# mpieva/mapping-iterative-assembler

Hardware: AMD Instinct MI355X
Metric: reads aligned/sec per iteration (16.5kb mito ref, 100bp reads) (higher is better)
Workload: dtype int32; 1 GPU; configs[1]: 1000000 synthetic 100 bp reads per GPU vs mt311 (16619 bp, circular), matrix flat; step = reiterate_assembly + pop_smp + cull + consensus; pass-1 coordinates = true positions; reads_per_gpu=1000000, total_reads=1000000, consensus_len=16619, bytes_per_read=182

## Files before the change

mapping-iterative-assembler_amd/csrc/align_body.h:

```cpp
#pragma once
#include "mia_layout.h"

namespace mia {

struct AlignArgs {
  const uint8_t* ref_codes;
  int32_t ref_start;
  int32_t len1;
  const uint8_t* read_packed;
  int32_t len2;
  const int32_t* pssm;
  int32_t sg5;
  PackParams pk;
  uint32_t lds_sub;
  uint32_t trace_stride;
  int16_t* cols_out;
  uint32_t dbg;
};

struct AlignResult {
  int32_t score, abc, abr, aec;
  uint32_t status;
  int32_t aer;
};

template <int CPL>
struct PackBits {
  static constexpr int IB = (CPL == 4) ? 8 : 10;
  static constexpr int SH = IB + 2;
  static constexpr uint32_t IDXM = (1u << IB) - 1u;
};

template <class P, int CPL, bool LASTCOL = false>
struct WindowAligner {
  typedef typename P::U U;
  typedef typename P::M M;
  static constexpr int IB = PackBits<CPL>::IB, SH = PackBits<CPL>::SH;
  static constexpr uint32_t IDXM = PackBits<CPL>::IDXM;

  MIA_HD static inline __attribute__((always_inline)) AlignResult run(P& w, const AlignArgs& a) {
    const uint32_t OFF = (uint32_t)a.pk.off;
    const uint32_t UNAV = ((uint32_t)a.pk.unavail << SH) | IDXM;
    const U lane = w.lane();
    const int len1 = a.len1, len2 = a.len2;
    const uint32_t RS2 = (uint32_t)((len2 + 1) & ~1) * 2u;

    for (int e0 = 0; e0 < len2 * 5; e0 += WAVE) {
      U e = lane + (uint32_t)e0;
      M ok = e < (uint32_t)(len2 * 5);
      U r = w.udiv5(e);
      U c1 = e - r * 5u;
      U byte = w.gload_u8(a.read_packed, r >> 1, ok);
      U c2 = (byte >> ((r & 1u) << 2)) & 15u;
      U d = w.depth(r, (uint32_t)len2);
      U v = w.gload_i32(a.pssm, (d * 5u + c1) * 5u + c2, ok);
      w.lds_w16(U(a.lds_sub) + c1 * RS2 + r * 2u, v, ok);
    }
    w.lds_fence();

    U col[CPL], sub_addr[CPL], KC[CPL], QC[CPL];
    for (int j = 0; j < CPL; j++) {
      col[j] = lane * (uint32_t)CPL + (uint32_t)j;
      M in = col[j] < (uint32_t)len1;
      U code = w.sel(in, w.gload_u8(a.ref_codes, U((uint32_t)a.ref_start) + col[j], in), U(4u));
      sub_addr[j] = U(a.lds_sub) + code * RS2;
      KC[j] = (U(0u) - ((U((uint32_t)GOP) + (col[j] - 1u) * (uint32_t)GEP) << SH)) + (TR_COLGAP << IB) + (col[j] - 1u - IDXM);
      QC[j] = ((col[j] * (uint32_t)GEP) << SH) + (U(IDXM) - col[j]);
    }
    const uint32_t WDC = TR_DIAG << IB;
    const U unav = U(UNAV);

    U Sb[CPL], q[CPL], rrun[CPL], pend[CPL], pw[CPL];
    {
      const uint32_t rk = IDXM;
      for (int j = 0; j < CPL; j++) {
        pw[j] = w.lds_r32(sub_addr[j]);
        Sb[j] = w.sext_lo(pw[j]) + OFF;
        q[j] = (Sb[j] << SH) + QC[j];
        pend[j] = (Sb[j] << SH) + rk;
        rrun[j] = unav;
      }
      for (int j4 = 0; j4 < CPL; j4 += 4)
        w.tr_w32(col[j4], U((TR_DIAG << 6) * 0x01010101u), col[j4] < (uint32_t)a.trace_stride);
    }
    U colbest = U(0u), colrow = U(0u);
    auto last_col_update = [&](int r) __attribute__((always_inline)) {
      U v = U(0u);
      for (int j = 0; j < CPL; j++) v = w.sel(col[j] == (uint32_t)(len1 - 1), Sb[j], v);
      M up = v > colbest;
      colbest = w.sel(up, v, colbest);
      colrow = w.sel(up, U((uint32_t)r), colrow);
    };
    if (LASTCOL) last_col_update(0);

    for (int r = 1; r < ((a.dbg & 4u) ? 1 : len2); r++) {
      const int32_t fresh = a.sg5 ? -(GOP + GEP * (r + 1)) : 0;
      const uint32_t freshb = (uint32_t)(fresh + (int32_t)OFF);
      const uint32_t WS = freshb << SH;
      const uint32_t KR = (0u - ((uint32_t)(GOP + GEP * (r - 1)) << SH)) + (TR_ROWGAP << IB) + ((uint32_t)(r - 1) - IDXM);
      const uint32_t RK = ((uint32_t)(GEP * r) << SH) + (IDXM - (uint32_t)r);
      const uint32_t row_tr = (uint32_t)r * a.trace_stride;
      const bool hi = (r & 1) != 0;
      if (!hi)
        for (int j = 0; j < CPL; j++) pw[j] = w.lds_r32(sub_addr[j] + (uint32_t)r * 2u);

      U dleft = w.shr1(Sb[CPL - 1], U(freshb));
      U rleft = w.shr1_max(rrun[CPL - 1], unav);
      U u0 = w.shr1_max(q[CPL - 2], unav);
      U u1 = w.shr1_max(q[CPL - 1], unav);
      U g[CPL];
      g[0] = u0;
      g[1] = w.umax(u0, u1);
      for (int j = 2; j < CPL; j++) g[j] = w.umax(g[j - 1], q[j - 2]);
      U excl = w.shr1_max(w.scan_max(g[CPL - 1]), unav);

      U best[CPL], Snew[CPL];
      for (int j = 0; j < CPL; j++) {
        U diag = (j == 0) ? dleft : Sb[j - 1];
        U rl = (j == 0) ? rleft : rrun[j - 1];
        U Wd = (diag << SH) + WDC;
        U Wc = w.umax(excl, g[j]) + KC[j];
        U Wr = rl + KR;
        U m3 = w.umax3(Wd, Wc, Wr);
        best[j] = w.umax(m3, U(WS));
        U sub = hi ? w.sext_hi(pw[j]) : w.sext_lo(pw[j]);
        Snew[j] = (best[j] >> SH) + w.sel(m3 < WS, U(0u), sub);
      }
// ... 79 lines not shown
```

mapping-iterative-assembler_amd/csrc/mia_hip.hip:

```cpp
#include <hip/hip_runtime.h>
#include <atomic>
#include <hip/hip_ext.h>
#include <stdio.h>
#include <stdlib.h>
#include <string.h>

#include <algorithm>
#include <cmath>
#include <chrono>
#include <string>
#include <thread>
#include <vector>

#include "../../include/mia_hip.h"
#include "mia_comm.h"
#include "mia_consensus_kernels.h"
#include "mia_kernels.h"
#include "bandx_kernels.h"
#include "mia_pass1_kernels.h"
#include "mia_myers_kernels.h"
#include "mia_trim_kernels.h"
#include "mia_peak_kernels.h"
#include "mia_iter_kernels.h"
#include "mia_ma_region_kernels.h"

using namespace mia;

enum Stage { STG_TRACE = 0, STG_PLAIN, STG_FILTER, STG_BAND, STG_BX_PLAN, STG_BX_VALUES, STG_BX_TRACE, STG_TALLY, STG_PASS1, STG_MA_SELECT, STG_MA_RENDER, STG_COUNT };
static const char* const STAGE_NAMES[STG_COUNT] = {"k_align_quad", "k_align_quad_plain", "k_diag_filter", "k_band_align", "k_bx_plan",
                                                   "k_bx_values", "k_bx_trace", "k_tally_binned", "k_pass1", "k_ma_region_select",
                                                   "k_ma_region_render"};

constexpr int OPEN_WGS = 1024;
constexpr int64_t OPEN_SLAB_BYTES = (int64_t)MAX_READ * 64 * 12;
constexpr int CTRL_BINS = 0;
constexpr int CTRL_HDR = (3 * N_BINS + 2 + 1) & ~1;
constexpr int CTRL_FILTER = CTRL_HDR + PH_WORDS;
constexpr int CTRL_LKN = CTRL_FILTER + 4, CTRL_CULLF = CTRL_LKN + 1, CTRL_NEV = CTRL_CULLF + 1, CTRL_TFLAGS = CTRL_NEV + 1;
constexpr int CTRL_GENN = CTRL_TFLAGS + 2;
constexpr int CTRL_BXC = (CTRL_GENN + 1 + 63) & ~63;
constexpr int CTRL_WORDS = CTRL_BXC + BXC_WORDS;
constexpr int CTRL_C0 = CTRL_BINS + 3 * N_BINS, CTRL_CN = CTRL_WORDS - CTRL_C0;

#ifdef MIA_HIP_ALT_PATHS
static inline const char* alt_env(const char* name) { return getenv(name); }
#define ALT_KERNEL(k) ((const void*)(k))
#else
static inline const char* alt_env(const char*) { return nullptr; }
#define ALT_KERNEL(k) ((const void*)nullptr)
#endif

struct mia_hip_ctx {
  int device = 0;
  int cus = 1;
  std::string err;
  struct PoolBlock { void* p; size_t cap; bool lent; };
  std::vector<PoolBlock> pool;
// ... 26 lines not shown
  int min_len = 0;
  std::vector<int32_t> h_len;
  uint64_t* d_rplanes = nullptr; int rplane_words = 0;
  int32_t* d_umax = nullptr; bool umax_valid = false;
  uint8_t* d_ref = nullptr; int ref_cap = 0; int L = 0, wrap = 0; int explicit_win = 0; bool have_ref = false; bool aligned = false;
  bool ref_mostly_bases = true;
  bool ref_few_n = true;
  int64_t kh_entries = 0;

  int32_t *d_bin_of = nullptr, *d_list = nullptr, *d_wide_list = nullptr, *d_retry_list = nullptr;
  int32_t* d_bins = nullptr;
  int32_t* d_plan_hdr = nullptr;
  bool deferred = false;
  unsigned char* d_slabs[N_CPL] = {nullptr, nullptr, nullptr};
  unsigned char* d_slabs_retry[3] = {nullptr, nullptr, nullptr};
  unsigned char* d_quad_slabs = nullptr;
  int quad_wgs = 0;
  int grid_wgs = 0;
  int window_wgs[N_CPL] = {0, 0, 0};
  int64_t plain_retried = 0, plain_total = 0;
  bool wide_to_caller = false;
  int32_t* d_scratch = nullptr; int64_t scratch_cap = 0; int64_t* d_scratch_off = nullptr; int64_t scratch_off_cap = 0;
  int32_t* d_open_list = nullptr; int64_t open_cap = 0; unsigned char* d_slabs_open = nullptr; bool use_direct_open = true; int64_t direct_open_steps = 0;
  bool direct_open_now = false;

  int use_filter = 1;
  int32_t *d_kocc_cnt = nullptr, *d_kocc_pos = nullptr;
  uint64_t* d_planes = nullptr; int64_t plane_cap = 0;
  uint32_t* d_filter_n = nullptr; int64_t filter_proven = 0, filter_seen = 0;
  int use_banddp = 1;
  int32_t* d_left_list = nullptr; int64_t left_cap = 0;
  uint32_t* d_band_slabs = nullptr; int64_t band_slab_cap = 0;
  int64_t band_done = 0;

  bool bx_ok = false;
  int use_bx = 1, use_lanes = 1; bool bx_serial = false; uint32_t bx_dbg = 0;
  int32_t *d_bx_sub = nullptr, *d_bx_mrow = nullptr; int16_t *d_bx_loss = nullptr, *d_bx_dl = nullptr;
  int32_t bx_min_m = 0, bx_max_m = 0;
  uint32_t* d_refnib = nullptr; int64_t refnib_cap = 0;
  uint32_t* d_khash = nullptr; int32_t* d_khash_ovf = nullptr; uint32_t khash_cap = 0;
  KbPair* d_kbits = nullptr;
  int use_quick = 1; int64_t quick_steps = 0;
  uint32_t* d_prep_bar = nullptr; uint32_t prep_bar_count = 0; bool no_prep_fuse = false;
  uint32_t* d_bx_plan = nullptr; int32_t* d_bx_expect = nullptr; int32_t* d_bx_lists = nullptr; int64_t bx_cap = 0;
  BxCandRec* d_bx_cand = nullptr; int64_t cand_cap = 0, cand2_cap = 0; bool plan_split = true;
  BxCandRec* d_bx_cand2 = nullptr; int use_fine = 1;
// ... 83 lines not shown
  mia_hip_collectives coll{}; bool comm = false; int comm_ranks = 1, comm_rank = 0; std::string coll_name;
  unsigned long long* d_gather = nullptr;
  std::vector<int64_t> h_gather;
  int64_t ev_pad = 0;
  int64_t* d_lstage = nullptr; int64_t lstage_cap = 0;
  int64_t* d_lmine = nullptr; int64_t lmine_cap = 0;
  int64_t* d_lall = nullptr; int64_t lall_cap = 0;
  int32_t* d_scores_all = nullptr; int64_t scores_all_cap = 0;
};

static void read_alt_switches(mia_hip_ctx* ctx) {
  auto on = [](const char* name) { const char* v = alt_env(name); return v && atoi(v) != 0; };
  if (on("MIA_HIP_NO_DIAG_FILTER")) { ctx->use_filter = 0; ctx->use_bx = 0; }
  if (on("MIA_HIP_NO_BAND_DP")) { ctx->use_banddp = 0; ctx->use_bx = 0; }
  if (on("MIA_HIP_NO_BANDX")) ctx->use_bx = 0;
  if (on("MIA_HIP_NO_LANES")) ctx->use_lanes = 0;
  if (on("MIA_HIP_BX_SERIAL")) ctx->bx_serial = true;
  if (on("MIA_HIP_NO_PLAN_SPLIT")) ctx->plan_split = false;
  if (on("MIA_HIP_NO_FINE")) ctx->use_fine = 0;
  if (const char* v = alt_env("MIA_HIP_FINE")) ctx->use_fine = atoi(v);
  if (on("MIA_HIP_NO_QUICK_PLAN")) ctx->use_quick = 0;
  if (const char* v = alt_env("MIA_HIP_QUICK_PLAN")) ctx->use_quick = atoi(v);
  if (on("MIA_HIP_NO_DIRECT_OPEN")) ctx->use_direct_open = false;
  if (on("MIA_HIP_NO_PREP_FUSE")) ctx->no_prep_fuse = true;
  if (on("MIA_HIP_NO_SPEC")) ctx->no_spec = true;
  if (on("MIA_HIP_SPEC_TEST")) ctx->spec_force = true;
  if (on("MIA_HIP_NO_SIDE_BUCKETS")) ctx->no_side_buckets = true;
  if (on("MIA_HIP_NO_ZERO_COPY")) ctx->zero_copy = false;
  if (on("MIA_HIP_NO_EXT_EVENTS")) ctx->ext_events = 0u;
  if (on("MIA_HIP_FAKE_EVENT_OVERFLOW")) ctx->fake_event_overflow = true;
  if (on("MIA_HIP_CULL_SCAN")) ctx->cull_scan = true;
  if (on("MIA_HIP_TAIL_SCANS")) ctx->tail_scans = true;
  if (on("MIA_HIP_NO_CULL_RECORDS")) ctx->cull_with_records = false;
  if (on("MIA_HIP_NO_BINNED_TALLY")) ctx->use_binned_tally = 0;
  if (on("MIA_HIP_NO_LINEAR_TALLY")) ctx->no_linear_tally = true;
  if (on("MIA_HIP_SORT2_UNPACKED")) ctx->sort2_unpacked = true;
  if (on("MIA_HIP_TALLY_INLINE")) ctx->tally_defer = false;
  if (const char* v = alt_env("MIA_HIP_STRAND_SPLIT")) ctx->tally_strand_split = atoi(v) != 0;
  if (on("MIA_HIP_NO_TALLY_RUNS")) ctx->tally_runs = false;
  if (on("MIA_HIP_NO_TALLY_RALL")) ctx->tally_rall = false;
  if (on("MIA_HIP_MYERS_NO_LANES")) ctx->myers_no_lanes = true;
  if (on("MIA_HIP_MYERS_NO_OND")) ctx->myers_no_ond = true;
  if (const char* v = alt_env("MIA_HIP_DEBUG_SKIP")) ctx->dbg = (uint32_t)atoi(v);
  if (const char* v = alt_env("MIA_HIP_BX_DEBUG")) ctx->bx_dbg = (uint32_t)atoi(v);
}

// ... 232 lines not shown
static void pack_reads(int64_t n, const char* bases, const int64_t* offsets, const uint32_t* roff, const uint16_t* len, uint8_t* packed) {
  uint8_t lut[256];
  for (int c = 0; c < 256; c++) lut[c] = base_code((char)c);
  auto range = [&](int64_t lo, int64_t hi) {
    for (int64_t i = lo; i < hi; i++) {
      const unsigned char* s = reinterpret_cast<const unsigned char*>(bases) + offsets[i];
      uint8_t* d = packed + roff[i];
      const int l = len[i];
      int k = 0;
      for (; k + 1 < l; k += 2) d[k >> 1] = (uint8_t)(lut[s[k]] | (lut[s[k + 1]] << 4));
      if (k < l) d[k >> 1] = lut[s[k]];
    }
  };
  int T = (int)std::thread::hardware_concurrency();
  if (const char* e = getenv("MIA_HIP_THREADS")) T = atoi(e);
  T = std::max(1, std::min(std::min(T, 32), (int)(n / 16384) + 1));
  if (T == 1) { range(0, n); return; }
  std::vector<std::thread> th;
  for (int t = 1; t < T; t++) th.emplace_back(range, n * t / T, n * (t + 1) / T);
  range(0, n / T);
  for (auto& x : th) x.join();
}

extern "C" int mia_hip_upload_reads(mia_hip_ctx* ctx, int64_t n, const char* bases, const int64_t* offsets, const uint8_t* rc,
                                    const uint8_t* strand_known, const int32_t* as, const int32_t* ae) {
  if (!ctx || n < 0 || (n > 0 && (!bases || !offsets || !rc || !strand_known || !as || !ae))) return MIA_HIP_ERR_ARG;
  if (n >= (int64_t)1 << 31) { ctx->err = "more than 2^31 reads per context"; return MIA_HIP_ERR_ARG; }
  HIPCHK(hipSetDevice(ctx->device));
  std::vector<uint32_t> roff((size_t)n);
  std::vector<uint16_t> len((size_t)n);
  uint64_t total = 0;
  int max_len = 1;
  for (int64_t i = 0; i < n; i++) {
    int64_t l = offsets[i + 1] - offsets[i];
    if (l < 1 || l > MIA_HIP_MAX_READ) { ctx->err = "read length outside 1..256 (INIT_ALN_SEQ_LEN)"; return MIA_HIP_ERR_ARG; }
    roff[i] = (uint32_t)total;
    len[i] = (uint16_t)l;
    if (l > max_len) max_len = (int)l;
    total += (uint64_t)(((l + 1) / 2 + 3) & ~3);
    if (total >= ((uint64_t)1 << 32)) { ctx->err = "packed read store exceeds 4 GiB per context"; return MIA_HIP_ERR_ARG; }
  }
  std::vector<uint8_t> packed((size_t)total + 8, 0);
  pack_reads(n, bases, offsets, roff.data(), len.data(), packed.data());
  ctx->max_len = max_len;
  ctx->min_len = max_len;
  ctx->h_len.assign(len.begin(), len.end());
// ... 14 lines not shown
  rcx |= dev_alloc(ctx, &ctx->d_cols, (size_t)n * stride);
  rcx |= dev_alloc(ctx, &ctx->d_bin_of, (size_t)n);
  rcx |= dev_alloc(ctx, &ctx->d_umax, (size_t)n);
  ctx->rplane_words = (max_len + 63) >> 6;
  rcx |= dev_alloc(ctx, &ctx->d_rplanes, (size_t)n * 2 * ctx->rplane_words + 2);
  rcx |= dev_alloc(ctx, &ctx->d_list, (size_t)n + 4 * N_BINS);
  rcx |= dev_alloc(ctx, &ctx->d_wide_list, (size_t)n);
  rcx |= dev_alloc(ctx, &ctx->d_retry_list, (size_t)n);
  rcx |= dev_alloc(ctx, &ctx->d_slot, (size_t)n);
  rcx |= dev_alloc(ctx, &ctx->d_partial, (size_t)(n / 256 + n / 4096 + 8));
  rcx |= dev_alloc(ctx, &ctx->d_drop_f, (size_t)n);
  rcx |= dev_alloc(ctx, &ctx->d_drop_b, (size_t)n);
  ctx->n_slots = 2 * n + 16;
  rcx |= dev_alloc(ctx, &ctx->d_slot_dropped, (size_t)ctx->n_slots);
  rcx |= dev_alloc(ctx, &ctx->d_back_slot, (size_t)n) | dev_alloc(ctx, &ctx->d_front_slot0, (size_t)n);
  rcx |= dev_alloc(ctx, &ctx->ri.flen, (size_t)n) | dev_alloc(ctx, &ctx->ri.blen, (size_t)n) | dev_alloc(ctx, &ctx->ri.actf, (size_t)n) |
         dev_alloc(ctx, &ctx->ri.trec, (size_t)n * 16);
  ctx->slot_cap = 2 * n + 16;
  rcx |= dev_alloc(ctx, &ctx->si.reclen, (size_t)ctx->slot_cap) | dev_alloc(ctx, &ctx->si.recact, (size_t)ctx->slot_cap) | dev_alloc(ctx, &ctx->si.writer, (size_t)ctx->slot_cap) |
         dev_alloc(ctx, &ctx->si.mult, (size_t)ctx->slot_cap);
  ctx->lk.cap = (int32_t)std::min<int64_t>(n + 16, (int64_t)1 << 20);
  if (ctx->lk.cap > (int32_t)LINK_NONE - 1) ctx->lk.cap = (int32_t)LINK_NONE - 1;
  rcx |= dev_alloc(ctx, &ctx->lk.rec, (size_t)ctx->lk.cap * 4);
  if (rcx) return MIA_HIP_ERR_NOMEM;
  HIPCHK(hipMemcpyAsync(ctx->d_packed, packed.data(), packed.size(), hipMemcpyHostToDevice, ctx->stream));
  HIPCHK(hipMemcpyAsync(ctx->d_roff, roff.data(), (size_t)n * 4, hipMemcpyHostToDevice, ctx->stream));
  HIPCHK(hipMemcpyAsync(ctx->d_len, len.data(), (size_t)n * 2, hipMemcpyHostToDevice, ctx->stream));
  HIPCHK(hipMemcpyAsync(ctx->d_rc, rc, (size_t)n, hipMemcpyHostToDevice, ctx->stream));
  HIPCHK(hipMemcpyAsync(ctx->d_sk, strand_known, (size_t)n, hipMemcpyHostToDevice, ctx->stream));
  HIPCHK(hipMemcpyAsync(ctx->d_as, as, (size_t)n * 4, hipMemcpyHostToDevice, ctx->stream));
  HIPCHK(hipMemcpyAsync(ctx->d_ae, ae, (size_t)n * 4, hipMemcpyHostToDevice, ctx->stream));
  HIPCHK(hipMemsetAsync(ctx->d_score, 0, (size_t)n * 4, ctx->stream));
  HIPCHK(hipMemsetAsync(ctx->d_status, 0, (size_t)n * 4, ctx->stream));
  HIPCHK(hipMemsetAsync(ctx->d_abr, 0, (size_t)n * 2, ctx->stream));
  HIPCHK(hipMemsetAsync(ctx->d_slot_dropped, 0, (size_t)ctx->n_slots, ctx->stream));
  HIPCHK(hipMemsetAsync(ctx->d_back_slot, 0xFF, (size_t)n * 8, ctx->stream));
  HIPCHK(hipMemsetAsync(ctx->d_front_slot0, 0xFF, (size_t)n * 8, ctx->stream));
  HIPCHK(hipMemsetAsync(ctx->d_drop_f, 0, (size_t)n, ctx->stream));
  HIPCHK(hipMemsetAsync(ctx->d_drop_b, 0, (size_t)n, ctx->stream));
  HIPCHK(hipStreamSynchronize(ctx->stream));
  ReadSet& r = ctx->rs;
  r.n = n; r.packed = ctx->d_packed; r.roff = ctx->d_roff; r.len = ctx->d_len; r.rc = ctx->d_rc; r.sk = ctx->d_sk;
  r.as = ctx->d_as; r.ae = ctx->d_ae; r.score = ctx->d_score; r.refstart = ctx->d_refstart; r.abr = ctx->d_abr;
  r.status = ctx->d_status; r.cols = ctx->d_cols; r.stride = stride;
  if (ctx->d_order) { (void)hipFree(ctx->d_order); ctx->d_order = nullptr; }
  if (ctx->d_order2) { (void)hipFree(ctx->d_order2); ctx->d_order2 = nullptr; }
// ... 200 lines not shown
  }
  RefInfo ref{ctx->d_ref, ctx->L, ctx->wrap, ctx->explicit_win};
  if (stage_begin(ctx, STG_TRACE, on)) return hipErrorOutOfMemory;
  launch_k(k_align_window<CPL>, dim3(grid), dim3(64), 0, on ? on : ctx->stream, stop, ctx->rs, ref, ctx->d_pssm, ctx->packs.p[ci], list,
           count, slabs, slab, ctx->d_wide_list, ctx->d_bins + 3 * N_BINS, ctx->dbg, dev_range);
  stage_end(ctx, STG_TRACE, on);
  return hipGetLastError();
}

static int bx_join_and_retry(mia_hip_ctx* ctx) {
  if (!ctx->bx_pending_join) return MIA_HIP_OK;
  ctx->bx_pending_join = false;
  const int32_t* range = ctx->d_plan_hdr + PH_RETRY2;
  const int cols = ctx->max_len + 2 * REALIGN_BUFFER + 2;
  const bool aside = ctx->bx_planner_aside;
  if (!aside || ctx->dp_aside) HIPCHK(hipStreamWaitEvent(ctx->stream, ctx->ev_join, 0));
  HIPCHK(hipStreamWaitEvent(ctx->stream, ctx->ev_join3, 0));
  hipEvent_t stop = (aside && (ctx->ext_events & 8u)) ? ctx->ev_fork : nullptr;
  ctx->align_end_signalled = stop != nullptr;
  hipError_t e;
  if (ctx->direct_open_now) {
    RefInfo ref{ctx->d_ref, ctx->L, ctx->wrap, ctx->explicit_win};
    if (stage_begin(ctx, STG_TRACE)) return MIA_HIP_ERR_NOMEM;
    launch_k(k_align_open, dim3(OPEN_WGS), dim3(64), 0, ctx->stream, stop, ctx->rs, ref, (const int32_t*)ctx->d_pssm, ctx->packs, (const int32_t*)ctx->d_open_list,
             (const uint32_t*)(ctx->d_bx_ctr + (size_t)BXC_OPEN * BXC_STRIDE), ctx->d_slabs_open, (int64_t)OPEN_SLAB_BYTES, ctx->d_wide_list, ctx->d_bins + 3 * N_BINS, ctx->dbg,
             (const int32_t*)ctx->d_retry2, (const uint32_t*)(range + 1));
    stage_end(ctx, STG_TRACE);
    e = hipGetLastError();
    if (e != hipSuccess) { ctx->err = std::string("k_align_open launch: ") + hipGetErrorString(e); return MIA_HIP_ERR_DEVICE; }
    return MIA_HIP_OK;
  }
  e = cols <= 64 * 4 ? launch_window<4>(ctx, 0, ctx->d_retry2, 0, range, nullptr, aside, stop)
    : cols <= 64 * 8 ? launch_window<8>(ctx, 1, ctx->d_retry2, 0, range, nullptr, aside, stop)
                     : launch_window<12>(ctx, 2, ctx->d_retry2, 0, range, nullptr, aside, stop);
  if (e != hipSuccess) { ctx->err = std::string("k_align_window (band retry list) launch: ") + hipGetErrorString(e); return MIA_HIP_ERR_DEVICE; }
  if (aside) {
    if (!ctx->planner_end_signalled) HIPCHK(hipEventRecord(ctx->ev_join, ctx->stream2));
    ctx->planner_end_signalled = false;
    HIPCHK(hipStreamWaitEvent(ctx->stream, ctx->ev_join, 0));
  }
  return MIA_HIP_OK;
}

static int align_all(mia_hip_ctx* ctx);
static bool tally_is_binned(const mia_hip_ctx* ctx);
static int comm_pre_cull_enqueue(mia_hip_ctx* ctx, const int32_t* d_wide_count);
static bool comm_pre_cull_collect(mia_hip_ctx* ctx);

extern "C" int mia_hip_realign(mia_hip_ctx* ctx, const char* new_ref, int32_t ref_len, int circular) {
// ... 233 lines not shown
      bd.rplanes = bd.umax ? ctx->d_rplanes : nullptr;
      bd.rplane_words = ctx->rplane_words;
      bd.plan = ctx->d_bx_plan; bd.expect = ctx->d_bx_expect; bd.lists = ctx->d_bx_lists; bd.list_stride = ctx->bx_cap; bd.ctr = ctx->d_bx_ctr;
      const bool split = ctx->plan_split;
      const bool fork_by_launch = (ctx->ext_events & 1u) && new_flow && !(ctx->dbg & 256u);
      bd.cand = nullptr; bd.cand_n = ctx->d_bx_ctr + (size_t)BXC_CAND * BXC_STRIDE;
      bd.cand2 = nullptr; bd.cand2_n = ctx->d_bx_ctr + (size_t)BXC_CAND2 * BXC_STRIDE;
      int64_t rejects_before = 0;
      for (int k = 1; k < BXF_KINDS; k++) rejects_before += ctx->bx_last[BXC_FAIL0 + k];
      const bool fine = split && ctx->use_fine && (ctx->use_fine > 1 || !ctx->flat || n >= 4000000 || !ctx->ref_mostly_bases || rejects_before * 20 > n);
      if (split) {
        if (n > ctx->cand_cap) {
          if (dev_alloc(ctx, &ctx->d_bx_cand, (size_t)n)) return MIA_HIP_ERR_NOMEM;
          ctx->cand_cap = n;
        }
        if (fine && n > ctx->cand2_cap) {
          if (dev_alloc(ctx, &ctx->d_bx_cand2, (size_t)n)) return MIA_HIP_ERR_NOMEM;
          ctx->cand2_cap = n;
        }
        bd.cand = ctx->d_bx_cand;
        if (fine) bd.cand2 = ctx->d_bx_cand2;
      }
      const int last_phase = split ? (fine ? 3 : 2) : 0;
      {
        int64_t lr = 0;
        for (int k = 1; k < BXF_KINDS; k++) lr += ctx->bx_last[BXC_FAIL0 + k];
        const bool many_early = !ctx->ref_mostly_bases || lr * 20 > n;
        planner_head_first = new_flow && ctx->deferred && many_early && !(ctx->dbg & 256u);
        const bool plain_wanted = many_early;
        direct_open = new_flow && ctx->deferred && ctx->use_direct_open && !plain_wanted && !planner_head_first && !(ctx->dbg & 256u) &&
                      !(ctx->bx_dbg & (4u | 8u));
      }
      bd.open = nullptr; bd.open_n = ctx->d_bx_ctr + (size_t)BXC_OPEN * BXC_STRIDE;
      ctx->direct_open_now = direct_open;
      if (direct_open) {
        if (n > ctx->open_cap) { if (dev_alloc(ctx, &ctx->d_open_list, (size_t)n)) return MIA_HIP_ERR_NOMEM; ctx->open_cap = n; }
        if (!ctx->d_slabs_open && hipMalloc((void**)&ctx->d_slabs_open, (size_t)OPEN_SLAB_BYTES * OPEN_WGS) != hipSuccess) return MIA_HIP_ERR_NOMEM;
        bd.open = ctx->d_open_list;
        ctx->direct_open_steps++;
      }
      if (!fine && ctx->use_fine < 2) bd.tab.maxw = 32;
      const bool quick = split && new_flow && want_bits && !(ctx->bx_dbg & 32u) && bd.umax != nullptr &&
                         (!fine || n >= 2000000 || ctx->use_quick > 1);
      bd.qlist = nullptr; bd.qlist_n = ctx->d_filter_n + 1; bd.mark_all = 0; bd.to_late = 0; bd.qch = 4;
      bool plan_launched = false;
      const bool fork_at_quick = quick && ctx->deferred && direct_open && !fine && !planner_head_first && !(ctx->bx_dbg & (4u | 8u));
      bd.kb = KmerBits{quick ? ctx->d_kbits : nullptr, ctx->L};
      const bool quick_lds = quick && words * 24 <= 38 * 1024;
      bd.plane_words = (int32_t)(quick_lds ? words : 0);
      if (quick) {
        if (n > ctx->left_cap) { if (dev_alloc(ctx, &ctx->d_left_list, (size_t)n)) return MIA_HIP_ERR_NOMEM; ctx->left_cap = n; }
        bd.qlist = ctx->d_left_list;
        ctx->quick_steps++;
      }
      if (stage_begin(ctx, STG_BX_PLAN)) return MIA_HIP_ERR_NOMEM;
      {
        const int32_t* in_list = quick ? ctx->d_left_list : nullptr;
        const dim3 pb(256);
        const int nwords = (ctx->max_len + 63) >> 6;
        const bool one_launch = quick && !fine;
        if (quick) {
          bd.qch = (n >= 4000000 && words * 24 <= 16 * 1024) ? BX_QCH : 4;
          const dim3 pg((unsigned)((n + 256 * bd.qch - 1) / (256 * bd.qch)));
          hipEvent_t done = (fork_at_quick && fork_by_launch) ? ctx->ev_fork : nullptr;
          const int32_t* in_list = nullptr;
#define MIA_PLAN(NWV, PHV) launch_k(k_bx_plan<NWV, PHV>, pg, pb, (size_t)(bx_quick_lds_words(bd.qch) * 8 + (PHV == 5 ? words * 24 : 0)), ctx->stream, done, ctx->rs, ref, rp, kh, (int64_t)wrap, bd, in_list, (const uint32_t*)(ctx->d_filter_n + 1), n, ctx->d_bin_of)
          if (quick_lds) { switch (nwords) { case 1: MIA_PLAN(1, 5); break; case 2: MIA_PLAN(2, 5); break; case 3: MIA_PLAN(3, 5); break; default: MIA_PLAN(4, 5); break; } }
          else { switch (nwords) { case 1: MIA_PLAN(1, 4); break; case 2: MIA_PLAN(2, 4); break; case 3: MIA_PLAN(3, 4); break; default: MIA_PLAN(4, 4); break; } }
#undef MIA_PLAN
          bd.mark_all = 1;
          if (fork_at_quick) {
            if (!fork_by_launch) HIPCHK(hipEventRecord(ctx->ev_fork, ctx->stream));
            bd.to_late = 1;
          }
        }
        const int phase_first = (split && !one_launch) ? 1 : 0, phase_last = one_launch ? 0 : last_phase;
        plan_launched = true;
        for (int phase = phase_first; phase <= phase_last; phase++) {
          const dim3 pg(phase >= 2 ? (unsigned)std::min<int64_t>((n + 255) / 256, 1024) : (unsigned)(one_launch ? std::min<int64_t>((n + 255) / 256, 256) : (n + 255) / 256));
          hipEvent_t done = (fork_by_launch && phase == phase_last && !planner_head_first && !fork_at_quick) ? ctx->ev_fork : nullptr;
#define MIA_PLAN(NWV, PHV) launch_k(k_bx_plan<NWV, PHV>, pg, pb, 0, ctx->stream, done, ctx->rs, ref, rp, kh, (int64_t)wrap, bd, in_list, (const uint32_t*)(ctx->d_filter_n + 1), n, ctx->d_bin_of)
#define MIA_PLAN_NW(PHV) switch (nwords) { case 1: MIA_PLAN(1, PHV); break; case 2: MIA_PLAN(2, PHV); break; case 3: MIA_PLAN(3, PHV); break; default: MIA_PLAN(4, PHV); break; }
          switch (phase) {
            case 0: if (one_launch) { MIA_PLAN_NW(6) } else { MIA_PLAN_NW(0) } break;
            case 1: MIA_PLAN_NW(1) break;
            case 2: MIA_PLAN_NW(2) break;
            default: MIA_PLAN_NW(3) break;
          }
#undef MIA_PLAN_NW
#undef MIA_PLAN
        }
        bd.to_late = 0;
      }
      stage_end(ctx, STG_BX_PLAN);
      HIPCHK(hipGetLastError());
      if (planner_head_first) {
        hipLaunchKernelGGL(k_plan_count, dim3(gb), dim3(tb), 0, ctx->stream, ctx->rs, ref, ctx->packs, 1, filtered, filtered, ctx->d_bin_of, d_count, ctx->d_filter_n);
        hipLaunchKernelGGL(k_plan_scan, dim3(1), dim3(512), 0, ctx->stream, d_count, d_off, ctx->d_plan_hdr, 0, ctx->d_list);
        launch_k(k_plan_fill, dim3(gb), dim3(tb), 0, ctx->stream, fork_by_launch ? ctx->ev_fork : nullptr, n, (const int32_t*)ctx->d_bin_of, (const int32_t*)d_off, d_cursor, ctx->d_list);
        HIPCHK(hipGetLastError());
      }
      if (!(ctx->dbg & 256u)) {
        if (new_flow) {
          hipStream_t vs = (ctx->deferred && !fork_at_quick) ? ctx->stream : ctx->stream2;
// ... 946 lines not shown
```

mapping-iterative-assembler_amd/csrc/mia_kernels.h:

```cpp
#pragma once
#include <hip/hip_runtime.h>
#include <stdint.h>

#include "align_body.h"
#include "align_body_quad.h"
#include "align_body_quad_plain.h"
#include "diag_filter.h"
#include "band_body.h"
#include "mia_layout.h"
#include "wave_dev.h"

namespace mia {

constexpr int N_CPL = 3;
constexpr int BIN_WIDE = N_CPL;
constexpr int BIN_QUAD0 = BIN_WIDE + 1;
constexpr int N_BINS = BIN_QUAD0 + MAX_READ + 1;
constexpr int SUB_LDS_BYTES = MAX_READ * 10;

struct ReadSet {
  int64_t n;
  const uint8_t* packed;
  const uint32_t* roff;
  const uint16_t* len;
// ... 340 lines not shown
    a.trace_stride = (uint32_t)((l1 + 3) & ~3);
    a.cols_out = rs.cols + (int64_t)i * rs.stride;
    a.dbg = dbg;
    AlignResult r = WindowAligner<DevWave, CPL>::run(wave, a);
    if (wave.lane() == 0) {
      if (r.status & ST_ESCAPE) {
        int p = atomicAdd(wide_count, 1);
        wide_list[p] = i;
      } else {
        rs.score[i] = r.score;
        rs.refstart[i] = s;
        rs.abr[i] = (int16_t)r.abr;
        rs.as[i] = r.abc + s;
        rs.ae[i] = r.aec + s;
      }
      rs.status[i] = r.status;
    }
    wave.lds_fence();
  }
}

__global__ __launch_bounds__(64) void k_align_open(ReadSet rs, RefInfo ref, const int32_t* pssm2, PackSet ps, const int32_t* list, const uint32_t* count_p,
                                                    unsigned char* trace_slabs, int64_t slab_bytes, int32_t* wide_list, int32_t* wide_count, uint32_t dbg,
                                                    const int32_t* list_b, const uint32_t* count_b_p) {
  __shared__ __attribute__((aligned(16))) unsigned char lds_raw[SUB_LDS_BYTES];
  const int count_a = (int)*count_p, count = count_a + (list_b ? (int)*count_b_p : 0);
  __builtin_amdgcn_s_setprio(3);
  DevWave wave(lds_raw, trace_slabs + (int64_t)blockIdx.x * slab_bytes);
  for (int w = blockIdx.x; w < count; w += gridDim.x) {
    const int i = w < count_a ? list[w] : list_b[w - count_a];
    if (!rs.sk[i]) { if (wave.lane() == 0) rs.status[i] = ST_SKIPPED; continue; }
    AlignArgs a;
    int s, l1;
    const int len2 = rs.len[i];
    read_window(ref, rs.as[i], rs.ae[i], len2, &s, &l1);
    const int ci = classify(len2, l1, ps, 0);
    if (ci == BIN_WIDE) {
      if (wave.lane() == 0) { const int q = atomicAdd(wide_count, 1); wide_list[q] = i; }
      continue;
    }
    a.ref_codes = ref.codes;
    a.ref_start = s;
    a.len1 = l1;
    a.read_packed = rs.packed + rs.roff[i];
    a.len2 = len2;
    a.pssm = pssm2 + (rs.rc[i] ? PSSM_WORDS : 0);
    a.sg5 = 1;
    a.pk = ps.p[ci];
    a.lds_sub = 0;
    a.trace_stride = (uint32_t)((l1 + 3) & ~3);
    a.cols_out = rs.cols + (int64_t)i * rs.stride;
    a.dbg = dbg;
    AlignResult r;
    if (ci == 0) r = WindowAligner<DevWave, 4>::run(wave, a);
    else if (ci == 1) r = WindowAligner<DevWave, 8>::run(wave, a);
    else r = WindowAligner<DevWave, 12>::run(wave, a);
    if (wave.lane() == 0) {
      if (r.status & ST_ESCAPE) {
        const int q = atomicAdd(wide_count, 1);
        wide_list[q] = i;
      } else {
        rs.score[i] = r.score;
        rs.refstart[i] = s;
        rs.abr[i] = (int16_t)r.abr;
        rs.as[i] = r.abc + s;
        rs.ae[i] = r.aec + s;
      }
      rs.status[i] = r.status;
    }
    wave.lds_fence();
  }
}

__global__ __launch_bounds__(64, 4) void k_align_quad(ReadSet rs, RefInfo ref, const int32_t* pssm2, PackParams pk, const int32_t* list,
                                                    int32_t n_quads, unsigned char* trace_slabs, int64_t slab_bytes,
                                                    int32_t* wide_list, int32_t* wide_count, int32_t* retry_list, int32_t* retry_count,
                                                    int32_t band, uint32_t dbg, const int32_t* dev_range) {
  extern __shared__ __attribute__((aligned(16))) unsigned char lds_raw[];
  if (dev_range) { list += dev_range[0]; n_quads = dev_range[1]; }
// ... 211 lines not shown
```

mapping-iterative-assembler_amd/csrc/wave_dev.h:

```cpp
#pragma once
#include <hip/hip_runtime.h>
#include <stdint.h>

#include "mia_layout.h"

namespace mia {

constexpr int DPP_ROW_SHR = 0x110;
constexpr int DPP_WAVE_SHR1 = 0x138;
constexpr int DPP_ROW_BCAST15 = 0x142;
constexpr int DPP_ROW_BCAST31 = 0x143;

struct DevWave {
  typedef uint32_t U;
  typedef bool M;
  unsigned char* lds;
  unsigned char* trace;

  __device__ __forceinline__ DevWave(unsigned char* l, unsigned char* t) : lds(l), trace(t) {}

  __device__ __forceinline__ U lane() const { return __builtin_amdgcn_mbcnt_hi(~0u, __builtin_amdgcn_mbcnt_lo(~0u, 0u)); }

  __device__ __forceinline__ U shr1(U x, U fill) const {
    return (U)__builtin_amdgcn_update_dpp((int)fill, (int)x, DPP_WAVE_SHR1, 0xF, 0xF, false);
// ... 122 lines not shown
  __device__ __forceinline__ U lds_r32m(U off, M ok) const { return ok ? *reinterpret_cast<const uint32_t*>(lds + off) : 0u; }
  __device__ __forceinline__ static U gload_u32(const uint32_t* p, U i, M ok) { return ok ? p[i] : 0u; }
  __device__ __forceinline__ static void gstore_u32(uint32_t* p, U i, U v, M ok) { if (ok) p[i] = v; }
  __device__ __forceinline__ U tr_r16(U off, M ok) const {
    return ok ? (U)__hip_atomic_load(reinterpret_cast<const uint16_t*>(trace + off), __ATOMIC_RELAXED, __HIP_MEMORY_SCOPE_AGENT) : 0u;
  }
  __device__ __forceinline__ void tr_w32(U off, U v, M ok) const { if (ok) *reinterpret_cast<uint32_t*>(trace + off) = v; }
  __device__ __forceinline__ U tr_r8(U off, M ok) const {
    return ok ? (U)__hip_atomic_load(trace + off, __ATOMIC_RELAXED, __HIP_MEMORY_SCOPE_AGENT) : 0u;
  }
  __device__ __forceinline__ void tr_fence() const {
    __builtin_amdgcn_fence(__ATOMIC_RELEASE, "workgroup");
    __builtin_amdgcn_wave_barrier();
    __builtin_amdgcn_fence(__ATOMIC_ACQUIRE, "workgroup");
  }
  __device__ __forceinline__ void sched_fence() const { __builtin_amdgcn_sched_barrier(0); }
  __device__ __forceinline__ void lds_fence() const {
    __builtin_amdgcn_fence(__ATOMIC_RELEASE, "workgroup");
    __builtin_amdgcn_wave_barrier();
    __builtin_amdgcn_fence(__ATOMIC_ACQUIRE, "workgroup");
  }
};

}
```

Baseline: 1.440 billion reads/s.

## Keep open-window traceback matrix in LDS and batch PSSM staging loads

The open-window alignment kernel now uses dynamic shared memory sized from the device limit, and narrow-bin reads whose traceback fits are written and read from LDS instead of a global slab. The substitution-staging loop batches eight rows of global loads before the LDS writes so more loads are in flight, and the per-row LDS substitution read is prefetched one row ahead. Global slabs are now sized by max read length and allocated at read upload, and an env flag forces all reads through the open path. The larger LDS footprint per workgroup may lower occupancy, and extra registers for the batching and prefetch may add register pressure.

```diff
diff --git a/mapping-iterative-assembler_amd/csrc/align_body.h b/mapping-iterative-assembler_amd/csrc/align_body.h
--- a/mapping-iterative-assembler_amd/csrc/align_body.h
+++ b/mapping-iterative-assembler_amd/csrc/align_body.h
@@ -31,7 +31,7 @@
   static constexpr uint32_t IDXM = (1u << IB) - 1u;
 };
 
-template <class P, int CPL, bool LASTCOL = false>
+template <class P, int CPL, bool LASTCOL = false, bool ALONE = false>
 struct WindowAligner {
   typedef typename P::U U;
   typedef typename P::M M;
@@ -45,32 +45,50 @@
     const int len1 = a.len1, len2 = a.len2;
     const uint32_t RS2 = (uint32_t)((len2 + 1) & ~1) * 2u;
 
-    for (int e0 = 0; e0 < len2 * 5; e0 += WAVE) {
-      U e = lane + (uint32_t)e0;
-      M ok = e < (uint32_t)(len2 * 5);
-      U r = w.udiv5(e);
-      U c1 = e - r * 5u;
-      U byte = w.gload_u8(a.read_packed, r >> 1, ok);
-      U c2 = (byte >> ((r & 1u) << 2)) & 15u;
-      U d = w.depth(r, (uint32_t)len2);
-      U v = w.gload_i32(a.pssm, (d * 5u + c1) * 5u + c2, ok);
-      w.lds_w16(U(a.lds_sub) + c1 * RS2 + r * 2u, v, ok);
+    U col[CPL], code[CPL];
+    auto load_codes = [&]() __attribute__((always_inline)) {
+      for (int j = 0; j < CPL; j++) {
+        col[j] = lane * (uint32_t)CPL + (uint32_t)j;
+        M in = col[j] < (uint32_t)len1;
+        code[j] = w.sel(in, w.gload_u8(a.ref_codes, U((uint32_t)a.ref_start) + col[j], in), U(4u));
+      }
+    };
+    if (ALONE) load_codes();
+
+    constexpr int SUB_BATCH = ALONE ? 8 : 1;
+    for (int e0 = 0; e0 < len2 * 5; e0 += SUB_BATCH * WAVE) {
+      U sr[SUB_BATCH], sc1[SUB_BATCH], sbyte[SUB_BATCH], sv[SUB_BATCH];
+      for (int k = 0; k < SUB_BATCH; k++) {
+        U e = lane + (uint32_t)(e0 + k * WAVE);
+        M ok = e < (uint32_t)(len2 * 5);
+        sr[k] = w.udiv5(e);
+        sc1[k] = e - sr[k] * 5u;
+        sbyte[k] = w.gload_u8(a.read_packed, sr[k] >> 1, ok);
+      }
+      for (int k = 0; k < SUB_BATCH; k++) {
+        M ok = (lane + (uint32_t)(e0 + k * WAVE)) < (uint32_t)(len2 * 5);
+        U c2 = (sbyte[k] >> ((sr[k] & 1u) << 2)) & 15u;
+        U d = w.depth(sr[k], (uint32_t)len2);
+        sv[k] = w.gload_i32(a.pssm, (d * 5u + sc1[k]) * 5u + c2, ok);
+      }
+      for (int k = 0; k < SUB_BATCH; k++) {
+        M ok = (lane + (uint32_t)(e0 + k * WAVE)) < (uint32_t)(len2 * 5);
+        w.lds_w16(U(a.lds_sub) + sc1[k] * RS2 + sr[k] * 2u, sv[k], ok);
+      }
     }
     w.lds_fence();
-
-    U col[CPL], sub_addr[CPL], KC[CPL], QC[CPL];
+    if (!ALONE) load_codes();
+
+    U sub_addr[CPL], KC[CPL], QC[CPL];
     for (int j = 0; j < CPL; j++) {
-      col[j] = lane * (uint32_t)CPL + (uint32_t)j;
-      M in = col[j] < (uint32_t)len1;
-      U code = w.sel(in, w.gload_u8(a.ref_codes, U((uint32_t)a.ref_start) + col[j], in), U(4u));
-      sub_addr[j] = U(a.lds_sub) + code * RS2;
+      sub_addr[j] = U(a.lds_sub) + code[j] * RS2;
       KC[j] = (U(0u) - ((U((uint32_t)GOP) + (col[j] - 1u) * (uint32_t)GEP) << SH)) + (TR_COLGAP << IB) + (col[j] - 1u - IDXM);
       QC[j] = ((col[j] * (uint32_t)GEP) << SH) + (U(IDXM) - col[j]);
     }
     const uint32_t WDC = TR_DIAG << IB;
     const U unav = U(UNAV);
 
-    U Sb[CPL], q[CPL], rrun[CPL], pend[CPL], pw[CPL];
+    U Sb[CPL], q[CPL], rrun[CPL], pend[CPL], pw[CPL], pwn[CPL];
     {
       const uint32_t rk = IDXM;
       for (int j = 0; j < CPL; j++) {
@@ -93,6 +111,7 @@
     };
     if (LASTCOL) last_col_update(0);
 
+    for (int j = 0; j < CPL; j++) pwn[j] = pw[j];
     for (int r = 1; r < ((a.dbg & 4u) ? 1 : len2); r++) {
       const int32_t fresh = a.sg5 ? -(GOP + GEP * (r + 1)) : 0;
       const uint32_t freshb = (uint32_t)(fresh + (int32_t)OFF);
@@ -101,8 +120,14 @@
       const uint32_t RK = ((uint32_t)(GEP * r) << SH) + (IDXM - (uint32_t)r);
       const uint32_t row_tr = (uint32_t)r * a.trace_stride;
       const bool hi = (r & 1) != 0;
-      if (!hi)
-        for (int j = 0; j < CPL; j++) pw[j] = w.lds_r32(sub_addr[j] + (uint32_t)r * 2u);
+      if (!ALONE) {
+        if (!hi)
+          for (int j = 0; j < CPL; j++) pw[j] = w.lds_r32(sub_addr[j] + (uint32_t)r * 2u);
+      } else if (!hi) {
+        for (int j = 0; j < CPL; j++) pw[j] = pwn[j];
+      } else if (r + 1 < len2) {
+        for (int j = 0; j < CPL; j++) pwn[j] = w.lds_r32(sub_addr[j] + (uint32_t)(r + 1) * 2u);
+      }
 
       U dleft = w.shr1(Sb[CPL - 1], U(freshb));
       U rleft = w.shr1_max(rrun[CPL - 1], unav);
diff --git a/mapping-iterative-assembler_amd/csrc/mia_hip.hip b/mapping-iterative-assembler_amd/csrc/mia_hip.hip
--- a/mapping-iterative-assembler_amd/csrc/mia_hip.hip
+++ b/mapping-iterative-assembler_amd/csrc/mia_hip.hip
@@ -32,7 +32,7 @@
                                                    "k_ma_region_render"};
 
 constexpr int OPEN_WGS = 1024;
-constexpr int64_t OPEN_SLAB_BYTES = (int64_t)MAX_READ * 64 * 12;
+constexpr int64_t OPEN_SLAB_ROW = 64 * 12;
 constexpr int CTRL_BINS = 0;
 constexpr int CTRL_HDR = (3 * N_BINS + 2 + 1) & ~1;
 constexpr int CTRL_FILTER = CTRL_HDR + PH_WORDS;
@@ -105,6 +105,8 @@
   bool wide_to_caller = false;
   int32_t* d_scratch = nullptr; int64_t scratch_cap = 0; int64_t* d_scratch_off = nullptr; int64_t scratch_off_cap = 0;
   int32_t* d_open_list = nullptr; int64_t open_cap = 0; unsigned char* d_slabs_open = nullptr; bool use_direct_open = true; int64_t direct_open_steps = 0;
+  int64_t open_slab_bytes = 0; int open_lds_trace = 0;
+  bool all_open = false;
   bool direct_open_now = false;
 
   int use_filter = 1;
@@ -234,6 +236,7 @@
   if (on("MIA_HIP_NO_QUICK_PLAN")) ctx->use_quick = 0;
   if (const char* v = alt_env("MIA_HIP_QUICK_PLAN")) ctx->use_quick = atoi(v);
   if (on("MIA_HIP_NO_DIRECT_OPEN")) ctx->use_direct_open = false;
+  if (on("MIA_HIP_ALL_OPEN")) ctx->all_open = true;
   if (on("MIA_HIP_NO_PREP_FUSE")) ctx->no_prep_fuse = true;
   if (on("MIA_HIP_NO_SPEC")) ctx->no_spec = true;
   if (on("MIA_HIP_SPEC_TEST")) ctx->spec_force = true;
@@ -512,6 +515,32 @@
   for (auto& x : th) x.join();
 }
 
+static int open_read_buffers(mia_hip_ctx* ctx) {
+  if (!ctx->use_direct_open) return MIA_HIP_OK;
+  hipDeviceProp_t prop;
+  int64_t cap = 64 * 1024;
+  if (hipGetDeviceProperties(&prop, ctx->device) == hipSuccess && (int64_t)prop.sharedMemPerBlock > cap) cap = (int64_t)prop.sharedMemPerBlock;
+  if (cap > 160 * 1024) cap = 160 * 1024;
+  const int len = ctx->max_len;
+  const int st0 = (len + 2 * REALIGN_BUFFER + 2 + 3) & ~3, st_wide = st0 + 32;
+  const int per4 = (int)(((cap / 4 - SUB_LDS_BYTES) / len) & ~3);
+  const int stride = st_wide <= per4 ? st_wide : (st0 <= per4 ? per4 : st0);
+  int64_t bytes = ((int64_t)stride * len + 15) & ~(int64_t)15;
+  if (bytes > cap / 2 - SUB_LDS_BYTES) bytes = (cap / 2 - SUB_LDS_BYTES) & ~(int64_t)15;
+  ctx->open_lds_trace = (int)bytes;
+  if (SUB_LDS_BYTES + bytes > 48 * 1024 &&
+      hipFuncSetAttribute((const void*)k_align_open, hipFuncAttributeMaxDynamicSharedMemorySize, (int)(SUB_LDS_BYTES + bytes)) != hipSuccess) {
+    (void)hipGetLastError();
+    ctx->open_lds_trace = 48 * 1024 - SUB_LDS_BYTES;
+  }
+  const int64_t slab = OPEN_SLAB_ROW * len;
+  if (slab != ctx->open_slab_bytes || !ctx->d_slabs_open) {
+    if (dev_alloc(ctx, &ctx->d_slabs_open, (size_t)(slab * OPEN_WGS))) return MIA_HIP_ERR_NOMEM;
+    ctx->open_slab_bytes = slab;
+  }
+  return MIA_HIP_OK;
+}
+
 extern "C" int mia_hip_upload_reads(mia_hip_ctx* ctx, int64_t n, const char* bases, const int64_t* offsets, const uint8_t* rc,
                                     const uint8_t* strand_known, const int32_t* as, const int32_t* ae) {
   if (!ctx || n < 0 || (n > 0 && (!bases || !offsets || !rc || !strand_known || !as || !ae))) return MIA_HIP_ERR_ARG;
@@ -572,6 +601,7 @@
   ctx->lk.cap = (int32_t)std::min<int64_t>(n + 16, (int64_t)1 << 20);
   if (ctx->lk.cap > (int32_t)LINK_NONE - 1) ctx->lk.cap = (int32_t)LINK_NONE - 1;
   rcx |= dev_alloc(ctx, &ctx->lk.rec, (size_t)ctx->lk.cap * 4);
+  rcx |= open_read_buffers(ctx);
   if (rcx) return MIA_HIP_ERR_NOMEM;
   HIPCHK(hipMemcpyAsync(ctx->d_packed, packed.data(), packed.size(), hipMemcpyHostToDevice, ctx->stream));
   HIPCHK(hipMemcpyAsync(ctx->d_roff, roff.data(), (size_t)n * 4, hipMemcpyHostToDevice, ctx->stream));
@@ -818,9 +848,9 @@
   if (ctx->direct_open_now) {
     RefInfo ref{ctx->d_ref, ctx->L, ctx->wrap, ctx->explicit_win};
     if (stage_begin(ctx, STG_TRACE)) return MIA_HIP_ERR_NOMEM;
-    launch_k(k_align_open, dim3(OPEN_WGS), dim3(64), 0, ctx->stream, stop, ctx->rs, ref, (const int32_t*)ctx->d_pssm, ctx->packs, (const int32_t*)ctx->d_open_list,
-             (const uint32_t*)(ctx->d_bx_ctr + (size_t)BXC_OPEN * BXC_STRIDE), ctx->d_slabs_open, (int64_t)OPEN_SLAB_BYTES, ctx->d_wide_list, ctx->d_bins + 3 * N_BINS, ctx->dbg,
-             (const int32_t*)ctx->d_retry2, (const uint32_t*)(range + 1));
+    launch_k(k_align_open, dim3(OPEN_WGS), dim3(64), (size_t)(SUB_LDS_BYTES + ctx->open_lds_trace), ctx->stream, stop, ctx->rs, ref, (const int32_t*)ctx->d_pssm, ctx->packs, (const int32_t*)ctx->d_open_list,
+             (const uint32_t*)(ctx->d_bx_ctr + (size_t)BXC_OPEN * BXC_STRIDE), ctx->d_slabs_open, ctx->open_slab_bytes, ctx->d_wide_list, ctx->d_bins + 3 * N_BINS, ctx->dbg,
+             (const int32_t*)ctx->d_retry2, (const uint32_t*)(range + 1), (int32_t)ctx->open_lds_trace);
     stage_end(ctx, STG_TRACE);
     e = hipGetLastError();
     if (e != hipSuccess) { ctx->err = std::string("k_align_open launch: ") + hipGetErrorString(e); return MIA_HIP_ERR_DEVICE; }
@@ -1100,10 +1130,11 @@
         if (fine) bd.cand2 = ctx->d_bx_cand2;
       }
       const int last_phase = split ? (fine ? 3 : 2) : 0;
+      const int64_t plan_nref = ctx->all_open ? 0 : (int64_t)wrap;
       {
         int64_t lr = 0;
         for (int k = 1; k < BXF_KINDS; k++) lr += ctx->bx_last[BXC_FAIL0 + k];
-        const bool many_early = !ctx->ref_mostly_bases || lr * 20 > n;
+        const bool many_early = (!ctx->ref_mostly_bases || lr * 20 > n) && !ctx->all_open;
         planner_head_first = new_flow && ctx->deferred && many_early && !(ctx->dbg & 256u);
         const bool plain_wanted = many_early;
         direct_open = new_flow && ctx->deferred && ctx->use_direct_open && !plain_wanted && !planner_head_first && !(ctx->dbg & 256u) &&
@@ -1113,7 +1144,7 @@
       ctx->direct_open_now = direct_open;
       if (direct_open) {
         if (n > ctx->open_cap) { if (dev_alloc(ctx, &ctx->d_open_list, (size_t)n)) return MIA_HIP_ERR_NOMEM; ctx->open_cap = n; }
-        if (!ctx->d_slabs_open && hipMalloc((void**)&ctx->d_slabs_open, (size_t)OPEN_SLAB_BYTES * OPEN_WGS) != hipSuccess) return MIA_HIP_ERR_NOMEM;
+        if (!ctx->d_slabs_open) { ctx->err = "k_align_open's trace slabs are made with the read store (mia_hip_upload_reads)"; return MIA_HIP_ERR_STATE; }
         bd.open = ctx->d_open_list;
         ctx->direct_open_steps++;
       }
@@ -1142,7 +1173,7 @@
           const dim3 pg((unsigned)((n + 256 * bd.qch - 1) / (256 * bd.qch)));
           hipEvent_t done = (fork_at_quick && fork_by_launch) ? ctx->ev_fork : nullptr;
           const int32_t* in_list = nullptr;
-#define MIA_PLAN(NWV, PHV) launch_k(k_bx_plan<NWV, PHV>, pg, pb, (size_t)(bx_quick_lds_words(bd.qch) * 8 + (PHV == 5 ? words * 24 : 0)), ctx->stream, done, ctx->rs, ref, rp, kh, (int64_t)wrap, bd, in_list, (const uint32_t*)(ctx->d_filter_n + 1), n, ctx->d_bin_of)
+#define MIA_PLAN(NWV, PHV) launch_k(k_bx_plan<NWV, PHV>, pg, pb, (size_t)(bx_quick_lds_words(bd.qch) * 8 + (PHV == 5 ? words * 24 : 0)), ctx->stream, done, ctx->rs, ref, rp, kh, plan_nref, bd, in_list, (const uint32_t*)(ctx->d_filter_n + 1), n, ctx->d_bin_of)
           if (quick_lds) { switch (nwords) { case 1: MIA_PLAN(1, 5); break; case 2: MIA_PLAN(2, 5); break; case 3: MIA_PLAN(3, 5); break; default: MIA_PLAN(4, 5); break; } }
           else { switch (nwords) { case 1: MIA_PLAN(1, 4); break; case 2: MIA_PLAN(2, 4); break; case 3: MIA_PLAN(3, 4); break; default: MIA_PLAN(4, 4); break; } }
 #undef MIA_PLAN
@@ -1157,7 +1188,7 @@
         for (int phase = phase_first; phase <= phase_last; phase++) {
           const dim3 pg(phase >= 2 ? (unsigned)std::min<int64_t>((n + 255) / 256, 1024) : (unsigned)(one_launch ? std::min<int64_t>((n + 255) / 256, 256) : (n + 255) / 256));
           hipEvent_t done = (fork_by_launch && phase == phase_last && !planner_head_first && !fork_at_quick) ? ctx->ev_fork : nullptr;
-#define MIA_PLAN(NWV, PHV) launch_k(k_bx_plan<NWV, PHV>, pg, pb, 0, ctx->stream, done, ctx->rs, ref, rp, kh, (int64_t)wrap, bd, in_list, (const uint32_t*)(ctx->d_filter_n + 1), n, ctx->d_bin_of)
+#define MIA_PLAN(NWV, PHV) launch_k(k_bx_plan<NWV, PHV>, pg, pb, 0, ctx->stream, done, ctx->rs, ref, rp, kh, plan_nref, bd, in_list, (const uint32_t*)(ctx->d_filter_n + 1), n, ctx->d_bin_of)
 #define MIA_PLAN_NW(PHV) switch (nwords) { case 1: MIA_PLAN(1, PHV); break; case 2: MIA_PLAN(2, PHV); break; case 3: MIA_PLAN(3, PHV); break; default: MIA_PLAN(4, PHV); break; }
           switch (phase) {
             case 0: if (one_launch) { MIA_PLAN_NW(6) } else { MIA_PLAN_NW(0) } break;
diff --git a/mapping-iterative-assembler_amd/csrc/mia_kernels.h b/mapping-iterative-assembler_amd/csrc/mia_kernels.h
--- a/mapping-iterative-assembler_amd/csrc/mia_kernels.h
+++ b/mapping-iterative-assembler_amd/csrc/mia_kernels.h
@@ -386,18 +386,20 @@
 
 __global__ __launch_bounds__(64) void k_align_open(ReadSet rs, RefInfo ref, const int32_t* pssm2, PackSet ps, const int32_t* list, const uint32_t* count_p,
                                                     unsigned char* trace_slabs, int64_t slab_bytes, int32_t* wide_list, int32_t* wide_count, uint32_t dbg,
-                                                    const int32_t* list_b, const uint32_t* count_b_p) {
-  __shared__ __attribute__((aligned(16))) unsigned char lds_raw[SUB_LDS_BYTES];
+                                                    const int32_t* list_b, const uint32_t* count_b_p, int32_t lds_trace_bytes) {
+  extern __shared__ __attribute__((aligned(16))) unsigned char lds_raw[];
   const int count_a = (int)*count_p, count = count_a + (list_b ? (int)*count_b_p : 0);
   __builtin_amdgcn_s_setprio(3);
   DevWave wave(lds_raw, trace_slabs + (int64_t)blockIdx.x * slab_bytes);
+  DevWaveLds wave_lds(lds_raw, lds_raw + SUB_LDS_BYTES);
   for (int w = blockIdx.x; w < count; w += gridDim.x) {
     const int i = w < count_a ? list[w] : list_b[w - count_a];
-    if (!rs.sk[i]) { if (wave.lane() == 0) rs.status[i] = ST_SKIPPED; continue; }
+    const int sk = rs.sk[i], len2 = rs.len[i], as = rs.as[i], ae = rs.ae[i], rc = rs.rc[i];
+    const uint32_t roff = rs.roff[i];
+    if (!sk) { if (wave.lane() == 0) rs.status[i] = ST_SKIPPED; continue; }
     AlignArgs a;
     int s, l1;
-    const int len2 = rs.len[i];
-    read_window(ref, rs.as[i], rs.ae[i], len2, &s, &l1);
+    read_window(ref, as, ae, len2, &s, &l1);
     const int ci = classify(len2, l1, ps, 0);
     if (ci == BIN_WIDE) {
       if (wave.lane() == 0) { const int q = atomicAdd(wide_count, 1); wide_list[q] = i; }
@@ -406,19 +408,20 @@
     a.ref_codes = ref.codes;
     a.ref_start = s;
     a.len1 = l1;
-    a.read_packed = rs.packed + rs.roff[i];
+    a.read_packed = rs.packed + roff;
     a.len2 = len2;
-    a.pssm = pssm2 + (rs.rc[i] ? PSSM_WORDS : 0);
+    a.pssm = pssm2 + (rc ? PSSM_WORDS : 0);
     a.sg5 = 1;
     a.pk = ps.p[ci];
     a.lds_sub = 0;
     a.trace_stride = (uint32_t)((l1 + 3) & ~3);
     a.cols_out = rs.cols + (int64_t)i * rs.stride;
     a.dbg = dbg;
+    const bool in_lds = ci < 2 && (int64_t)a.trace_stride * len2 <= (int64_t)lds_trace_bytes;
     AlignResult r;
-    if (ci == 0) r = WindowAligner<DevWave, 4>::run(wave, a);
-    else if (ci == 1) r = WindowAligner<DevWave, 8>::run(wave, a);
-    else r = WindowAligner<DevWave, 12>::run(wave, a);
+    if (ci == 0) r = in_lds ? WindowAligner<DevWaveLds, 4, false, true>::run(wave_lds, a) : WindowAligner<DevWave, 4, false, true>::run(wave, a);
+    else if (ci == 1) r = in_lds ? WindowAligner<DevWaveLds, 8, false, true>::run(wave_lds, a) : WindowAligner<DevWave, 8, false, true>::run(wave, a);
+    else r = WindowAligner<DevWave, 12, false, true>::run(wave, a);
     if (wave.lane() == 0) {
       if (r.status & ST_ESCAPE) {
         const int q = atomicAdd(wide_count, 1);
diff --git a/mapping-iterative-assembler_amd/csrc/wave_dev.h b/mapping-iterative-assembler_amd/csrc/wave_dev.h
--- a/mapping-iterative-assembler_amd/csrc/wave_dev.h
+++ b/mapping-iterative-assembler_amd/csrc/wave_dev.h
@@ -168,4 +168,12 @@
   }
 };
 
+struct DevWaveLds : DevWave {
+  unsigned char* ltrace;
+  __device__ __forceinline__ DevWaveLds(unsigned char* l, unsigned char* lt) : DevWave(l, nullptr), ltrace(lt) {}
+  __device__ __forceinline__ void tr_w32(U off, U v, M ok) const { if (ok) *reinterpret_cast<uint32_t*>(ltrace + off) = v; }
+  __device__ __forceinline__ U tr_r8(U off, M ok) const { return ok ? (U)ltrace[off] : 0u; }
+  __device__ __forceinline__ void tr_fence() const { lds_fence(); }
+};
+
 }
```

New measurement: 1.451 billion reads/s, median of 6. About the same (+0.7%).
